# google/automl

Measured on NVIDIA H100. Metric: EfficientDet-D0 images/sec @ batch 32/GPU (640x640, forward + post-process), higher is better.
Workload: dtype f16 storage / f32 accumulate

## Files before the change

automl_b200/csrc/mbconv_fused.cu:

```cuda
#include "tc_common.cuh"

namespace edet {
namespace mbf {

using namespace pwtc;

constexpr int kThreads = 256;
constexpr int kPatch = 16;
constexpr int kPatchPx = kPatch * kPatch;
constexpr int kMaxCh = 64;
constexpr int kNT = kMaxCh / 16;
constexpr int kEPitch = kMaxCh * 2 + 16;

__device__ __forceinline__ uint32_t lds_b32(uint32_t addr) {
  uint32_t v;
  asm volatile("ld.shared.b32 %0, [%1];" : "=r"(v) : "r"(addr));
  return v;
}
__device__ __forceinline__ void sts_v4(uint32_t addr, const uint4& v) {
  asm volatile("st.shared.v4.b32 [%0], {%1, %2, %3, %4};" ::"r"(addr), "r"(v.x), "r"(v.y),
               "r"(v.z), "r"(v.w)
               : "memory");
}
__device__ __forceinline__ float2 h2_bits_to_f2(uint32_t v) {
  return __half22float2(*reinterpret_cast<const __half2*>(&v));
}

struct Params {
  int n, h, w, cin, cmid, ho, wo, pad_t, pad_l;
  int block_k, num_k_blocks, a_bytes, b_bytes, desc_sbo, desc_layout;
  int ch, num_chunks;
  int oth, otw;
  int tiles_y, tiles_x, total_tiles;
  const float* bias_e;
  const float* wd;
  const float* bias_d;
  __half* out;
  long long* se_sum;
  unsigned* sched;
};

struct Tile {
  int n, ty, tx, chunk;
};
__device__ __forceinline__ Tile decode(int t, const Params& p) {
  Tile r;
  r.chunk = t % p.num_chunks;
  t /= p.num_chunks;
  r.tx = t % p.tiles_x;
  t /= p.tiles_x;
  r.ty = t % p.tiles_y;
  r.n = t / p.tiles_y;
  return r;
}

template <int K, int S, int ACT, bool HAS_SE>
__global__ void __launch_bounds__(kThreads, 2)
mbconv_front_kernel(const __grid_constant__ CUtensorMap map_x,
                    const __grid_constant__ CUtensorMap map_w, const Params p) {
  constexpr int OTW = (kPatch - K) / S + 1;
  constexpr int NIX = (OTW - 1) * S + K;
  pdl_launch_dependents();
  extern __shared__ __align__(1024) uint8_t smem_raw[];
  uint8_t* smem = reinterpret_cast<uint8_t*>(
      (reinterpret_cast<uintptr_t>(smem_raw) + 1023) & ~static_cast<uintptr_t>(1023));
  uint8_t* smem_a = smem;
  uint8_t* smem_b = smem_a + p.a_bytes;
  uint8_t* smem_e = smem_b + p.b_bytes;
  unsigned long long* se_s =
      reinterpret_cast<unsigned long long*>(smem_e + kPatchPx * kEPitch);
  uint64_t* bars = reinterpret_cast<uint64_t*>(se_s + p.ch);
  const uint32_t full_bar = smem_u32(bars);
  volatile int* next_tile_s = reinterpret_cast<volatile int*>(bars + 1);

  const int warp = threadIdx.x >> 5, lane = threadIdx.x & 31;
  const int wg = warp >> 2;
  if (threadIdx.x == 0) {
    mbar_init(full_bar, 1);
    asm volatile("fence.mbarrier_init.release.cluster;" ::: "memory");
    asm volatile("prefetch.tensormap [%0];" ::"l"(reinterpret_cast<uint64_t>(&map_x)) : "memory");
    asm volatile("prefetch.tensormap [%0];" ::"l"(reinterpret_cast<uint64_t>(&map_w)) : "memory");
  }
  __syncthreads();
  pdl_wait_prior();

  const uint32_t tx_bytes = static_cast<uint32_t>(kPatchPx * p.block_k * 2 + p.ch * p.block_k * 2);
  const int pitch = p.block_k * 2;
  const int nt = p.ch >> 4;
  uint32_t full_phase = 0;

  auto issue_loads = [&](const Tile& tl, int kb) {
    mbar_expect_tx(full_bar, tx_bytes);
    tma_load_4d(smem_u32(smem_a), &map_x, full_bar, kb * p.block_k, tl.tx * OTW * S - p.pad_l,
                tl.ty * OTW * S - p.pad_t, tl.n);
    tma_load_3d(smem_u32(smem_b), &map_w, full_bar, kb * p.block_k, tl.chunk * p.ch, 0);
  };

  bool prefetched = false;
  int t = blockIdx.x;
  for (int it = 0; t < p.total_tiles; ++it) {
    const Tile tl = decode(t, p);
    const int cbase = tl.chunk * p.ch;
    const int cv = min(p.ch, p.cmid - cbase);
    float acc[2][kNT][8] = {};
    for (int kb = 0; kb < p.num_k_blocks; ++kb) {
      if (threadIdx.x == 0 && !(kb == 0 && prefetched)) issue_loads(tl, kb);
      mbar_wait(full_bar, full_phase);
      full_phase ^= 1;
      const int k_rem = p.cin - kb * p.block_k;
      const int ksteps = k_rem >= p.block_k ? p.block_k / MMA_K : (k_rem + MMA_K - 1) / MMA_K;
      const uint64_t db = make_smem_desc(smem_u32(smem_b), p.desc_sbo, p.desc_layout);
      wg_fence();
#pragma unroll
      for (int h = 0; h < 2; ++h) {
        const uint64_t da =
            make_smem_desc(smem_u32(smem_a + (wg * 128 + h * 64) * pitch), p.desc_sbo, p.desc_layout);
        wg_mma_kblock<kNT>(acc[h], da, db, pitch, nt, ksteps, kb == 0);
      }
      wg_commit();
      wg_wait<0>();
      __syncthreads();
    }
    wg_fence_acc<kNT>(acc[0]);
    wg_fence_acc<kNT>(acc[1]);
    if (threadIdx.x == 0) {
      const int tn = sched_next_tile(p.sched, p.total_tiles);
      next_tile_s[it & 1] = tn;
      prefetched = tn < p.total_tiles;
      if (prefetched) issue_loads(decode(tn, p), 0);
    }
    {
      const int cq = 2 * (lane & 3);
      const float* be = p.bias_e + cbase;
#pragma unroll
      for (int h = 0; h < 2; ++h) {
#pragma unroll
        for (int r = 0; r < 2; ++r) {
          const int m = wg * 128 + h * 64 + 16 * (warp & 3) + (lane >> 2) + 8 * r;
          const int py = m / kPatch, px = m % kPatch;
          const int iy = tl.ty * OTW * S - p.pad_t + py, ix = tl.tx * OTW * S - p.pad_l + px;
          const bool inside = iy >= 0 && iy < p.h && ix >= 0 && ix < p.w;
          const uint32_t erow = smem_u32(smem_e) + m * kEPitch;
#pragma unroll
          for (int j = 0; j < kNT; ++j) {
            const int col = 16 * j + cq;
            if (16 * j >= cv) continue;
            const bool hi_ok = 16 * j + 8 < cv;
            uint32_t lo_bits = 0u, hi_bits = 0u;
            if (inside) {
              const float2 b_lo = __ldg(reinterpret_cast<const float2*>(be + col));
              const float2 b_hi = hi_ok ? __ldg(reinterpret_cast<const float2*>(be + col + 8))
                                        : make_float2(0.f, 0.f);
              float2 lo = fadd2_rn(make_float2(acc[h][j][2 * r], acc[h][j][2 * r + 1]), b_lo);
              float2 hi = fadd2_rn(make_float2(acc[h][j][4 + 2 * r], acc[h][j][4 + 2 * r + 1]), b_hi);
              apply_act4<ACT>(lo, hi);
              const __half2 l2 = __floats2half2_rn(lo.x, lo.y), h2 = __floats2half2_rn(hi.x, hi.y);
              lo_bits = *reinterpret_cast<const uint32_t*>(&l2);
              hi_bits = *reinterpret_cast<const uint32_t*>(&h2);
            }
            asm volatile("st.shared.b32 [%0], %1;" ::"r"(erow + col * 2), "r"(lo_bits) : "memory");
            if (hi_ok)
              asm volatile("st.shared.b32 [%0], %1;" ::"r"(erow + (col + 8) * 2), "r"(hi_bits) : "memory");
          }
        }
      }
      if (HAS_SE)
        for (int i = threadIdx.x; i < p.ch; i += kThreads) se_s[i] = 0ull;
    }
    __syncthreads();
    {
      const int cpn = cv >> 1;
      const int oy0 = tl.ty * OTW, ox0 = tl.tx * OTW;
      const int rows = min(OTW, p.ho - oy0), cols = min(OTW, p.wo - ox0);
      const int cm2 = p.cmid >> 1;
      const uint32_t e_u32 = smem_u32(smem_e);
      if constexpr (K == 3 && S == 2) {
        constexpr int CG = 2;
        constexpr int NCG = (OTW + CG - 1) / CG;
        constexpr int IN_R = (OTW - 1) * S + K, IN_C = (CG - 1) * S + K;
        for (int item = threadIdx.x; item < NCG * cpn; item += kThreads) {
          const int xg = item / cpn, cp = item - xg * cpn;
          const float2* wd2 = reinterpret_cast<const float2*>(p.wd) + ((cbase >> 1) + cp);
          float2 wk[K * K];
#pragma unroll
          for (int i = 0; i < K * K; ++i) wk[i] = __ldg(wd2 + i * cm2);
          uint32_t coff[IN_C];
#pragma unroll
          for (int j = 0; j < IN_C; ++j)
            coff[j] = e_u32 + static_cast<uint32_t>(min(xg * CG * S + j, kPatch - 1) * kEPitch + cp * 4);
          float2 acc[OTW][CG];
#pragma unroll
          for (int r = 0; r < OTW; ++r)
#pragma unroll
            for (int tx = 0; tx < CG; ++tx) acc[r][tx] = make_float2(0.f, 0.f);
#pragma unroll
          for (int ir = 0; ir < IN_R; ++ir) {
            float2 xv[IN_C];
#pragma unroll
            for (int j = 0; j < IN_C; ++j) xv[j] = h2_bits_to_f2(lds_b32(coff[j] + ir * kPatch * kEPitch));
#pragma unroll
            for (int r = 0; r < OTW; ++r) {
              const int ky = ir - r * S;
              if (ky >= 0 && ky < K) {
#pragma unroll
                for (int tx = 0; tx < CG; ++tx)
#pragma unroll
                  for (int kx = 0; kx < K; ++kx)
                    acc[r][tx] = ffma2_rn(xv[tx * S + kx], wk[ky * K + kx], acc[r][tx]);
              }
            }
          }
          const float2 bd = __ldg(reinterpret_cast<const float2*>(p.bias_d + cbase) + cp);
          __half2* ocol = reinterpret_cast<__half2*>(p.out) +
                          ((static_cast<size_t>(tl.n) * p.ho + oy0) * p.wo + ox0 + xg * CG) * cm2 +
                          (cbase >> 1) + cp;
          float2 ssum = make_float2(0.f, 0.f);
#pragma unroll
          for (int r = 0; r < OTW; ++r) {
            float2 o0 = fadd2_rn(acc[r][0], bd), o1 = fadd2_rn(acc[r][1], bd);
            apply_act4<ACT>(o0, o1);
            if (r < rows) {
              if (xg * CG < cols) {
                if (HAS_SE) ssum = fadd2_rn(ssum, o0);
                ocol[static_cast<size_t>(r) * p.wo * cm2] = __floats2half2_rn(o0.x, o0.y);
              }
              if (xg * CG + 1 < cols) {
                if (HAS_SE) ssum = fadd2_rn(ssum, o1);
                ocol[static_cast<size_t>(r) * p.wo * cm2 + cm2] = __floats2half2_rn(o1.x, o1.y);
              }
            }
          }
          if (HAS_SE) {
            atomicAdd(&se_s[2 * cp], static_cast<unsigned long long>(__float2ll_rn(ssum.x * 1048576.f)));
            atomicAdd(&se_s[2 * cp + 1], static_cast<unsigned long long>(__float2ll_rn(ssum.y * 1048576.f)));
          }
        }
      } else {
      for (int item = threadIdx.x; item < rows * cpn; item += kThreads) {
        const int oyl = item / cpn, cp = item - oyl * cpn;
        const float2* wd2 = reinterpret_cast<const float2*>(p.wd) + ((cbase >> 1) + cp);
        const uint32_t ebase = e_u32 + (oyl * S * kPatch) * kEPitch + cp * 4;
        float2 acc[OTW];
#pragma unroll
        for (int i = 0; i < OTW; ++i) acc[i] = make_float2(0.f, 0.f);
#pragma unroll
        for (int ky = 0; ky < K; ++ky) {
          float2 wk[K];
#pragma unroll
          for (int kx = 0; kx < K; ++kx) wk[kx] = __ldg(wd2 + (ky * K + kx) * cm2);
#pragma unroll
          for (int ixl = 0; ixl < NIX; ++ixl) {
            const float2 v = h2_bits_to_f2(lds_b32(ebase + (ky * kPatch + ixl) * kEPitch));
#pragma unroll
            for (int kx = 0; kx < K; ++kx) {
              if ((ixl - kx) >= 0 && (ixl - kx) % S == 0 && (ixl - kx) / S < OTW)
                acc[(ixl - kx) / S] = ffma2_rn(v, wk[kx], acc[(ixl - kx) / S]);
            }
          }
        }
        const float2 bd = __ldg(reinterpret_cast<const float2*>(p.bias_d + cbase) + cp);
        __half2* orow = reinterpret_cast<__half2*>(p.out) +
                        ((static_cast<size_t>(tl.n) * p.ho + oy0 + oyl) * p.wo + ox0) * cm2 +
                        (cbase >> 1) + cp;
#pragma unroll
        for (int i = 0; i < OTW; ++i) acc[i] = fadd2_rn(acc[i], bd);
#pragma unroll
        for (int i = 0; i + 1 < OTW; i += 2) apply_act4<ACT>(acc[i], acc[i + 1]);
        if (OTW & 1) acc[OTW - 1] = apply_act2<ACT>(acc[OTW - 1]);
        float2 ssum = make_float2(0.f, 0.f);
#pragma unroll
        for (int oxl = 0; oxl < OTW; ++oxl) {
          if (oxl < cols) {
            if (HAS_SE) ssum = fadd2_rn(ssum, acc[oxl]);
            orow[static_cast<size_t>(oxl) * cm2] = __floats2half2_rn(acc[oxl].x, acc[oxl].y);
          }
        }
        if (HAS_SE) {
          atomicAdd(&se_s[2 * cp], static_cast<unsigned long long>(__float2ll_rn(ssum.x * 1048576.f)));
          atomicAdd(&se_s[2 * cp + 1], static_cast<unsigned long long>(__float2ll_rn(ssum.y * 1048576.f)));
        }
      }
      }
      if (HAS_SE) {
        __syncthreads();
        unsigned long long* dst = reinterpret_cast<unsigned long long*>(p.se_sum) +
                                  static_cast<size_t>(tl.n) * p.cmid + cbase;
        for (int i = threadIdx.x; i < cv; i += kThreads)
          if (se_s[i] != 0ull) atomicAdd(dst + i, se_s[i]);
      }
    }
    __syncthreads();
    t = next_tile_s[it & 1];
  }
}

template <int K, int S>
static int launch(const CUtensorMap& mx, const CUtensorMap& mw, const Params& p, int grid,
                  int smem_bytes, int act, bool has_se, cudaStream_t stream) {
#define EDET_MBF(ACT, SE)                                                                     \
  do {                                                                                        \
    auto kern = mbconv_front_kernel<K, S, ACT, SE>;                                           \
    static int configured[kMaxDevices];                                                       \
    if (int rc = ensure_dynamic_smem(kern, 232448, configured)) return rc;                    \
    EDET_CHECK_CUDA(launch_pdl(kern, dim3(grid), dim3(kThreads), smem_bytes, stream, mx, mw, p)); \
    return EDET_OK;                                                                           \
  } while (0)
  if (act == EDET_ACT_SWISH && has_se) EDET_MBF(EDET_ACT_SWISH, true);
  if (act == EDET_ACT_SWISH && !has_se) EDET_MBF(EDET_ACT_SWISH, false);
  if (act == EDET_ACT_RELU6 && has_se) EDET_MBF(EDET_ACT_RELU6, true);
  if (act == EDET_ACT_RELU6 && !has_se) EDET_MBF(EDET_ACT_RELU6, false);
#undef EDET_MBF
  set_error("mbconv_expand_dw: unsupported activation %d", act);
  return EDET_ERR_UNSUPPORTED;
}

}
}

extern "C" int edet_mbconv_expand_dw(const edet_half* x, const edet_half* we, const float* bias_e,
                                     const float* wd, const float* bias_d, edet_half* out,
                                     int64_t* se_sum, int n, int h, int w, int cin, int cmid,
                                     int k, int stride, int act, edet_stream_t stream) {
  using namespace edet;
  using namespace edet::mbf;
  EDET_CHECK_ARG(x && we && bias_e && wd && bias_d && out, "mbconv_expand_dw: null pointer");
  EDET_CHECK_ARG(n > 0 && h > 0 && w > 0 && cin % 8 == 0 && cmid % 8 == 0,
                 "mbconv_expand_dw: cin %% 8 and cmid %% 8 required (got %d, %d)", cin, cmid);
  EDET_CHECK_ARG((k == 3 || k == 5) && (stride == 1 || stride == 2), "mbconv_expand_dw: k/stride");
  Params p;
  p.n = n; p.h = h; p.w = w; p.cin = cin; p.cmid = cmid;
  p.ho = ceil_div(h, stride); p.wo = ceil_div(w, stride);
  p.pad_t = same_pad_before(h, k, stride); p.pad_l = same_pad_before(w, k, stride);
  p.num_chunks = ceil_div(cmid, kMaxCh);
  p.ch = ((ceil_div(cmid, p.num_chunks) + 15) / 16) * 16;
  p.oth = p.otw = (kPatch - k) / stride + 1;
  p.tiles_y = ceil_div(p.ho, p.oth); p.tiles_x = ceil_div(p.wo, p.otw);
  p.total_tiles = n * p.tiles_y * p.tiles_x * p.num_chunks;
  int smem_bytes = 0;
  for (int bk = cin <= 16 ? 16 : (cin <= 32 ? 32 : 64); bk >= 16; bk >>= 1) {
    p.block_k = bk;
    p.a_bytes = kPatchPx * bk * 2;
    p.b_bytes = ((p.ch * bk * 2 + 1023) / 1024) * 1024;
    smem_bytes = 1024 + p.a_bytes + p.b_bytes + kPatchPx * kEPitch + p.ch * 8 + 64;
    if (smem_bytes <= 113 * 1024 || bk == 32) break;
  }
  p.num_k_blocks = ceil_div(cin, p.block_k);
  p.desc_layout = desc_layout_for(p.block_k);
  p.desc_sbo = 8 * p.block_k * 2;
  p.bias_e = bias_e; p.bias_d = bias_d;
  p.wd = wd;
  p.out = reinterpret_cast<__half*>(out);
  p.se_sum = reinterpret_cast<long long*>(se_sum);
  p.sched = next_sched_slot();
  if (!p.sched) return EDET_ERR_CUDA;
  EDET_CHECK_ARG(smem_bytes <= 232448, "mbconv_expand_dw: tile needs %d bytes of smem", smem_bytes);
  CUtensorMap mx, mw;
  int rc;
  if ((rc = make_map4(&mx, x, cin, w, h, n, p.block_k, kPatch, kPatch))) return rc;
  if ((rc = make_map(&mw, we, cin, cmid, 1, cin, static_cast<uint64_t>(cmid) * cin, p.ch, p.block_k)))
    return rc;
  const int sm_count = device_sm_count();
  if (!sm_count) return EDET_ERR_CUDA;
  int per_sm = 232448 / (smem_bytes + 1024);
  if (per_sm < 1) per_sm = 1;
  if (per_sm > 2) per_sm = 2;
  const int grid = p.total_tiles < per_sm * sm_count ? p.total_tiles : per_sm * sm_count;
  const bool has_se = se_sum != nullptr;
  cudaStream_t s = as_stream(stream);
  if (k == 3 && stride == 1) return launch<3, 1>(mx, mw, p, grid, smem_bytes, act, has_se, s);
  if (k == 3 && stride == 2) return launch<3, 2>(mx, mw, p, grid, smem_bytes, act, has_se, s);
  if (k == 5 && stride == 1) return launch<5, 1>(mx, mw, p, grid, smem_bytes, act, has_se, s);
  return launch<5, 2>(mx, mw, p, grid, smem_bytes, act, has_se, s);
}
```

automl_b200/engine.py:

```python
import math
import os

import numpy as np
import torch

from automl_b200 import anchors as anchors_lib
from automl_b200 import ops
from automl_b200 import utils
from automl_b200.arch import DetArch


def _round_up(x, m):
  return (x + m - 1) // m * m


def _bn_fold(w, scope, eps):
  g = np.asarray(w[scope + '/gamma'], np.float64)
  b = np.asarray(w[scope + '/beta'], np.float64)
  m = np.asarray(w[scope + '/moving_mean'], np.float64)
  v = np.asarray(w[scope + '/moving_variance'], np.float64)
  scale = g / np.sqrt(v + eps)
  return scale, b - m * scale


def nms_v5_params(nms_configs):
  method = nms_configs['method']
  if method == 'hard' or not method:
    sigma = 0.0
    iou_thresh = nms_configs['iou_thresh'] or 0.5
    score_thresh = nms_configs['score_thresh'] or float('-inf')
  elif method == 'gaussian':
    sigma = nms_configs['sigma'] or 0.5
    iou_thresh = 0.5
    score_thresh = nms_configs['score_thresh'] or 0.001
  else:
    raise ValueError('Inference has invalid nms method {}'.format(method))
  return iou_thresh, score_thresh, sigma / 2


class Engine(object):

  def __init__(self, config, weights, batch_size, device='cuda:0', pw_impl=ops.PW_TCGEN05,
               use_cuda_graph=True, image_id_base=0, fuse_mbconv_front=False,
               fuse_sepconv=True, pipeline=True, defer_heads=False,
               fuse_class_argmax=True):
    if not torch.cuda.is_available():
      raise RuntimeError('automl_b200.Engine needs a CUDA device; there is no CPU fallback')
    self.config = config
    self.arch = a = DetArch(config)
    self.n = int(batch_size)
    self.device = torch.device(device)
    self.pw_impl = pw_impl
    self.use_cuda_graph = use_cuda_graph
    self.image_id_base = image_id_base
    if os.environ.get('EDET_FUSE_FRONT'):
      fuse_mbconv_front = os.environ['EDET_FUSE_FRONT'] != '0'
    self.fuse_mbconv_front = fuse_mbconv_front
    self.fuse_sepconv = fuse_sepconv
    if os.environ.get('EDET_PIPELINE'):
      pipeline = os.environ['EDET_PIPELINE'] != '0'
    self.pipeline = pipeline
    if os.environ.get('EDET_DEFER_HEADS'):
      defer_heads = os.environ['EDET_DEFER_HEADS'] != '0'
    self.defer_heads = bool(defer_heads and pipeline)
    self._deferred = None
    if os.environ.get('EDET_FUSE_ARGMAX'):
      fuse_class_argmax = os.environ['EDET_FUSE_ARGMAX'] != '0'
    self.fuse_class_argmax = fuse_class_argmax
    self._fused_target = None
    self._logits_current = False
    self.act = utils.activation_code(a.act_type)
    self._graph = None
    self._bb_split = None
    self._cell0_end = None
    self._ops = []
    self.op_info = []
    self._branch = None
    self._branch_streams = {}
    self.buffers = {}
    self._keep = []
    self.launches_per_forward = 0
    with torch.cuda.device(self.device):
      self._build(weights)

  def _dev(self, arr, dtype):
    t = torch.as_tensor(np.ascontiguousarray(arr)).to(dtype).to(self.device).contiguous()
    self._keep.append(t)
    return t

  def _buf(self, name, shape, dtype=torch.float16):
    t = torch.empty(shape, dtype=dtype, device=self.device)
    self.buffers[name] = t
    return t

  def _add(self, name, fn, kind='other', nbytes=0, flops=0, kernels=1, branch=None, needs=None):
    self._ops.append((name, fn))
    if branch is None:
      branch = self._branch
    self.op_info.append({'name': name, 'kind': kind, 'bytes': int(nbytes), 'flops': int(flops),
                         'kernels': int(kernels), 'branch': branch, 'needs': list(needs or [])})

  def _pw(self, name, a, wt, bias, out, act, residual=None, batch=1, rows=None, nout=None,
          branch=None):
    if rows is None:
      rows = a.numel() // (a.shape[-1] * batch)
    impl = self.pw_impl
    k = wt.shape[-1]
    n_out = nout if nout is not None else wt.shape[-2]
    m = rows * batch
    wbatch = wt.shape[0] if wt.dim() == 3 else 1
    nbytes = 2 * (m * k + m * n_out * (2 if residual is not None else 1)) + 2 * wbatch * n_out * k
    self._add(name, lambda: ops.pointwise_conv(a, wt, bias, out, act, residual=residual,
                                               rows=rows, batch=batch, nout=nout, impl=impl),
              kind='pointwise_tc' if impl == ops.PW_TCGEN05 else 'pointwise_simt',
              nbytes=nbytes, flops=2 * m * k * n_out, branch=branch)

  def _build(self, w):
    a, n, act = self.arch, self.n, self.act
    eps = a.bn_eps
    f16, f32 = torch.float16, torch.float32
    H, W = a.image_hw
    self.input = self._buf('input', (n, H, W, 3), f32)

    def check_c(c, what):
      if c % 8:
        raise NotImplementedError('%s has %d channels; the kernels need multiples of 8' % (what, c))

    bb = a.backbone_name
    scale, shift = _bn_fold(w, bb + '/stem/tpu_batch_normalization', eps)
    k = np.asarray(w[bb + '/stem/conv2d/kernel'], np.float64) * scale
    stem_w = self._dev(k.reshape(27, -1), f16)
    stem_b = self._dev(shift, f32)
    h, wd = a.level_hw[1]
    x = self._buf('stem', (n, h, wd, a.stem_filters))
    inp = self.input
    self._add('stem', lambda inp=inp, x=x: ops.stem_conv(inp, x, stem_w, stem_b, act),
              kind='stem', nbytes=12 * n * H * W + 2 * n * h * wd * a.stem_filters,
              flops=2 * 27 * n * h * wd * a.stem_filters)
    cur, cur_hw = x, (h, wd)

    feats = {}
    max_mid = max(b.mid_filters for b in a.blocks)
    se_acc = [self._buf('se_acc%d' % i, (n, max_mid), torch.int64) for i in range(2)]
    for t in se_acc:
      t.zero_()
    se_index = 0
    if any(b.se_filters for b in a.blocks):
      self._add('se_clear', lambda t=se_acc[0]: t.zero_(), kind='memset', nbytes=8 * n * max_mid,
                kernels=0)
    for b in a.blocks:
      scope = '%s/%s' % (bb, b.name)
      check_c(b.input_filters, scope); check_c(b.mid_filters, scope); check_c(b.output_filters, scope)
      h, wd = cur_hw
      x_in = cur
      mid = x_in
      fuse_front = (self.fuse_mbconv_front and b.expand_name and b.kernel_size == 3 and
                    b.stride == 2 and b.input_filters <= 64 and h * wd >= 1600)
      exp_wt = exp_b = None
      if b.expand_name:
        s, sh = _bn_fold(w, '%s/%s' % (scope, b.expand_bn), eps)
        kw = np.asarray(w['%s/%s/kernel' % (scope, b.expand_name)], np.float64)[0, 0]
        exp_wt = self._dev((kw * s).T, f16)
        exp_b = self._dev(sh, f32)
        if not fuse_front:
          mid = self._buf(b.name + '/expand', (n, h, wd, b.mid_filters))
          self._pw(b.name + '/expand', x_in, exp_wt, exp_b, mid, act)
      s, sh = _bn_fold(w, '%s/%s' % (scope, b.dw_bn), eps)
      kd = np.asarray(w[scope + '/depthwise_conv2d/depthwise_kernel'], np.float64)[..., 0]
      dw_w = self._dev((kd * s).reshape(b.kernel_size * b.kernel_size, -1), f32)
      dw_b = self._dev(sh, f32)
      ho, wo = utils.same_pad(h, b.kernel_size, b.stride)[0], utils.same_pad(wd, b.kernel_size, b.stride)[0]
      dwo = self._buf(b.name + '/dw', (n, ho, wo, b.mid_filters))
      partial = None
      if b.se_filters:
        partial = se_acc[se_index % 2].view(-1)[:n * b.mid_filters].view(n, b.mid_filters)
        next_zero = se_acc[(se_index + 1) % 2]
        se_index += 1
      if fuse_front:
        self._add(b.name + '/expand_dw',
                  lambda x_in=x_in, exp_wt=exp_wt, exp_b=exp_b, dwo=dwo, dw_w=dw_w, dw_b=dw_b,
                  partial=partial, b=b:
                  ops.mbconv_expand_dw(x_in, exp_wt, exp_b, dw_w, dw_b, dwo, act, b.kernel_size,
                                       b.stride, partial),
                  kind='mbconv_expand_dw',
                  nbytes=2 * n * (h * wd * b.input_filters + ho * wo * b.mid_filters)
                  + 2 * b.mid_filters * (b.input_filters + b.kernel_size**2)
                  + (8 * partial.numel() if partial is not None else 0),
                  flops=2 * n * b.mid_filters * (h * wd * b.input_filters + b.kernel_size**2 * ho * wo))
      else:
        self._add(b.name + '/dw',
                  lambda mid=mid, dwo=dwo, dw_w=dw_w, dw_b=dw_b, partial=partial, b=b:
                  ops.depthwise_conv(mid, dwo, dw_w, dw_b, act, b.kernel_size, b.stride, partial),
                  kind='depthwise_k%ds%d' % (b.kernel_size, b.stride),
                  nbytes=2 * n * b.mid_filters * (h * wd + ho * wo) + 2 * b.kernel_size**2 * b.mid_filters
                  + (8 * partial.numel() if partial is not None else 0),
                  flops=2 * b.kernel_size**2 * n * b.mid_filters * ho * wo)
      s, sh = _bn_fold(w, '%s/%s' % (scope, b.project_bn), eps)
      kp = np.asarray(w['%s/%s/kernel' % (scope, b.project_name)], np.float64)[0, 0]
      proj_wt = self._dev((kp * s).T, f16)
      proj_b = self._dev(sh, f32)
      y = self._buf(b.name + '/out', (n, ho, wo, b.output_filters))
      res = x_in if b.has_skip else None
      if b.reduction and b.reduction >= a.config.min_level and self._bb_split is None:
        self._bb_split = len(self._ops) + (1 if b.se_filters else 0)
      if b.se_filters:
        w1 = self._dev(np.asarray(w[scope + '/se/conv2d/kernel'], np.float64)[0, 0].T, f32)
        b1 = self._dev(w[scope + '/se/conv2d/bias'], f32)
        w2 = self._dev(np.asarray(w[scope + '/se/conv2d_1/kernel'], np.float64)[0, 0], f32)
        b2 = self._dev(w[scope + '/se/conv2d_1/bias'], f32)
        gate = self._buf(b.name + '/se_gate', (n, b.mid_filters), f32)
        hidden = self._buf(b.name + '/se_hidden', (n, b.se_filters), f32)
        wt_scaled = self._buf(b.name + '/proj_w', (n, b.output_filters, b.mid_filters))
        inv_hw = 1.0 / float(ho * wo)
        self._add(b.name + '/se',
                  lambda partial=partial, inv_hw=inv_hw, w1=w1, b1=b1, w2=w2, b2=b2, gate=gate,
                  proj_wt=proj_wt, wt_scaled=wt_scaled, next_zero=next_zero, hidden=hidden:
                  ops.se_fc(partial, inv_hw, w1, b1, w2, b2, gate, act, proj_wt, wt_scaled,
                            next_zero, hidden),
                  kind='se_fc', nbytes=8 * partial.numel() + 2 * proj_wt.numel() + 2 * wt_scaled.numel(),
                  kernels=2)
        self._pw(b.name + '/project', dwo, wt_scaled, proj_b, y, utils.ACT_NONE, residual=res,
                 batch=n, rows=ho * wo)
      else:
        self._pw(b.name + '/project', dwo, proj_wt, proj_b, y, utils.ACT_NONE, residual=res)
      cur, cur_hw = y, (ho, wo)
      if b.reduction:
        feats[b.reduction] = y

    self.num_backbone_ops = len(self._ops)
    if self._bb_split is None:
      self._bb_split = self.num_backbone_ops
    if self.defer_heads:
      for level in sorted(feats):
        if level >= a.config.min_level:
          src = feats[level]
          dst = self._buf('P%d_copy' % level, tuple(src.shape))
          self._add('feat_copy/P%d' % level, lambda src=src, dst=dst: dst.copy_(src),
                    kind='memcpy', nbytes=4 * src.numel(), kernels=0)
          feats[level] = dst
    self._heads_start = len(self._ops)
# ... 559 lines not shown
```

Baseline: 5237.

## Rework fused expand+depthwise kernel as streaming bands with ring buffer, enable auto fusion

Replaces the 16x16 patch tiling of the fused expand-pointwise + depthwise kernel with vertical strips processed as row bands. A double-buffered TMA pipeline feeds WGMMA, and expanded rows live in a shared-memory ring, so halo rows are not recomputed between bands. The host picks strip width and segment count to fit two CTAs per SM and balance the persistent grid. The engine now defaults to an automatic rule that turns the fusion on for large stride-2 k3 blocks, where previously it was off. This adds complexity and risks slowdowns where the fused path beats separate kernels less often than the rule assumes.

```diff
diff --git a/automl_b200/csrc/mbconv_fused.cu b/automl_b200/csrc/mbconv_fused.cu
--- a/automl_b200/csrc/mbconv_fused.cu
+++ b/automl_b200/csrc/mbconv_fused.cu
@@ -6,32 +6,36 @@
 using namespace pwtc;
 
 constexpr int kThreads = 256;
-constexpr int kPatch = 16;
-constexpr int kPatchPx = kPatch * kPatch;
-constexpr int kMaxCh = 64;
-constexpr int kNT = kMaxCh / 16;
-constexpr int kEPitch = kMaxCh * 2 + 16;
-
-__device__ __forceinline__ uint32_t lds_b32(uint32_t addr) {
-  uint32_t v;
-  asm volatile("ld.shared.b32 %0, [%1];" : "=r"(v) : "r"(addr));
-  return v;
-}
-__device__ __forceinline__ void sts_v4(uint32_t addr, const uint4& v) {
-  asm volatile("st.shared.v4.b32 [%0], {%1, %2, %3, %4};" ::"r"(addr), "r"(v.x), "r"(v.y),
-               "r"(v.z), "r"(v.w)
-               : "memory");
-}
-__device__ __forceinline__ float2 h2_bits_to_f2(uint32_t v) {
-  return __half22float2(*reinterpret_cast<const __half2*>(&v));
-}
+constexpr int kCh = 64;
+constexpr int kNT = kCh / 16;
+constexpr int kBK = 16;
+constexpr int kRowBytes = kBK * 2;
+constexpr int kBlockBytes = 64 * kRowBytes;
+constexpr int kEPitch = kCh * 2 + 16;
+constexpr int kTwoPerSm = 113 * 1024;
+constexpr int kMaxSmem = 232448;
+
+template <int K, int S>
+struct Cfg {
+  static constexpr int TR = (S == 2) ? 4 : (K == 3 ? 8 : 4);
+  static constexpr int TC = (S == 2) ? 2 : 4;
+  static constexpr int NR = TR * S;
+  static constexpr int HALO = K - S;
+  static constexpr int L = NR + HALO;
+  static constexpr int IN_COLS = (TC - 1) * S + K;
+  static constexpr int SW_MAX = S == 2 ? 32 : 64;
+  static constexpr int QMAX = (SW_MAX / TC * (kCh / 2) + kThreads - 1) / kThreads;
+};
 
 struct Params {
   int n, h, w, cin, cmid, ho, wo, pad_t, pad_l;
-  int block_k, num_k_blocks, a_bytes, b_bytes, desc_sbo, desc_layout;
-  int ch, num_chunks;
-  int oth, otw;
-  int tiles_y, tiles_x, total_tiles;
+  int nkb;
+  int sw, iw;
+  float inv_iw;
+  int m_blocks;
+  int a_bytes, w_bytes;
+  int nb;
+  int bands, strips, segs, chunks, total_units;
   const float* bias_e;
   const float* wd;
   const float* bias_d;
@@ -40,268 +44,305 @@
   unsigned* sched;
 };
 
-struct Tile {
-  int n, ty, tx, chunk;
+struct Unit {
+  int n, seg, strip, chunk;
 };
-__device__ __forceinline__ Tile decode(int t, const Params& p) {
-  Tile r;
-  r.chunk = t % p.num_chunks;
-  t /= p.num_chunks;
-  r.tx = t % p.tiles_x;
-  t /= p.tiles_x;
-  r.ty = t % p.tiles_y;
-  r.n = t / p.tiles_y;
+__device__ __forceinline__ Unit decode(int u, const Params& p) {
+  Unit r;
+  r.chunk = u % p.chunks;
+  u /= p.chunks;
+  r.strip = u % p.strips;
+  u /= p.strips;
+  r.seg = u % p.segs;
+  r.n = u / p.segs;
   return r;
+}
+
+__device__ __forceinline__ uint32_t lds_b32(uint32_t addr) {
+  uint32_t v;
+  asm volatile("ld.shared.b32 %0, [%1];" : "=r"(v) : "r"(addr));
+  return v;
+}
+__device__ __forceinline__ void sts_b32(uint32_t addr, uint32_t v) {
+  asm volatile("st.shared.b32 [%0], %1;" ::"r"(addr), "r"(v) : "memory");
 }
 
 template <int K, int S, int ACT, bool HAS_SE>
 __global__ void __launch_bounds__(kThreads, 2)
 mbconv_front_kernel(const __grid_constant__ CUtensorMap map_x,
                     const __grid_constant__ CUtensorMap map_w, const Params p) {
-  constexpr int OTW = (kPatch - K) / S + 1;
-  constexpr int NIX = (OTW - 1) * S + K;
+  using C = Cfg<K, S>;
+  constexpr int TR = C::TR, TC = C::TC, NR = C::NR, HALO = C::HALO, L = C::L;
+  constexpr int IN_COLS = C::IN_COLS;
   pdl_launch_dependents();
   extern __shared__ __align__(1024) uint8_t smem_raw[];
   uint8_t* smem = reinterpret_cast<uint8_t*>(
       (reinterpret_cast<uintptr_t>(smem_raw) + 1023) & ~static_cast<uintptr_t>(1023));
   uint8_t* smem_a = smem;
-  uint8_t* smem_b = smem_a + p.a_bytes;
-  uint8_t* smem_e = smem_b + p.b_bytes;
-  unsigned long long* se_s =
-      reinterpret_cast<unsigned long long*>(smem_e + kPatchPx * kEPitch);
-  uint64_t* bars = reinterpret_cast<uint64_t*>(se_s + p.ch);
-  const uint32_t full_bar = smem_u32(bars);
-  volatile int* next_tile_s = reinterpret_cast<volatile int*>(bars + 1);
-
-  const int warp = threadIdx.x >> 5, lane = threadIdx.x & 31;
+  uint8_t* smem_w = smem_a + 2 * p.a_bytes;
+  uint8_t* smem_e = smem_w + 2 * p.w_bytes;
+  const int ring_row_bytes = p.iw * kEPitch;
+  ulonglong2* se_s = reinterpret_cast<ulonglong2*>(smem_e + L * ring_row_bytes);
+  uint64_t* bars = reinterpret_cast<uint64_t*>(se_s + C::QMAX * kThreads);
+  volatile int* unit_s = reinterpret_cast<volatile int*>(bars + 2);
+
+  const int warp = __shfl_sync(0xffffffffu, static_cast<int>(threadIdx.x >> 5), 0);
+  const int lane = threadIdx.x & 31;
   const int wg = warp >> 2;
   if (threadIdx.x == 0) {
-    mbar_init(full_bar, 1);
+    mbar_init(smem_u32(&bars[0]), 1);
+    mbar_init(smem_u32(&bars[1]), 1);
     asm volatile("fence.mbarrier_init.release.cluster;" ::: "memory");
     asm volatile("prefetch.tensormap [%0];" ::"l"(reinterpret_cast<uint64_t>(&map_x)) : "memory");
     asm volatile("prefetch.tensormap [%0];" ::"l"(reinterpret_cast<uint64_t>(&map_w)) : "memory");
   }
+  pdl_wait_prior();
+
+  auto issue = [&](const Unit& un, int j, int stage, int wbuf) {
+    const uint32_t bar = smem_u32(&bars[stage]);
+    const uint32_t a_tx = static_cast<uint32_t>(p.nkb * NR * p.iw * kRowBytes);
+    mbar_expect_tx(bar, a_tx + (wbuf >= 0 ? static_cast<uint32_t>(p.nkb * kBlockBytes) : 0u));
+    const int y0 = (un.seg * p.nb * TR) * S - p.pad_t + HALO + (j - 1) * NR;
+    const int x0 = un.strip * p.sw * S - p.pad_l;
+    uint8_t* dst = smem_a + stage * p.a_bytes;
+    for (int kb = 0; kb < p.nkb; ++kb)
+      tma_load_4d(smem_u32(dst + kb * p.m_blocks * kBlockBytes), &map_x, bar, kb * kBK, x0, y0, un.n);
+    if (wbuf >= 0)
+      for (int kb = 0; kb < p.nkb; ++kb)
+        tma_load_3d(smem_u32(smem_w + wbuf * p.w_bytes + kb * kBlockBytes), &map_w, bar, kb * kBK,
+                    un.chunk * kCh, 0);
+  };
+  auto bands_of = [&](const Unit& un) { return min(p.nb, p.bands - un.seg * p.nb); };
+
+  if (threadIdx.x == 0) {
+    const int u0 = static_cast<int>(blockIdx.x);
+    unit_s[0] = u0;
+    issue(decode(u0, p), 0, 0, 0);
+  }
   __syncthreads();
-  pdl_wait_prior();
-
-  const uint32_t tx_bytes = static_cast<uint32_t>(kPatchPx * p.block_k * 2 + p.ch * p.block_k * 2);
-  const int pitch = p.block_k * 2;
-  const int nt = p.ch >> 4;
-  uint32_t full_phase = 0;
-
-  auto issue_loads = [&](const Tile& tl, int kb) {
-    mbar_expect_tx(full_bar, tx_bytes);
-    tma_load_4d(smem_u32(smem_a), &map_x, full_bar, kb * p.block_k, tl.tx * OTW * S - p.pad_l,
-                tl.ty * OTW * S - p.pad_t, tl.n);
-    tma_load_3d(smem_u32(smem_b), &map_w, full_bar, kb * p.block_k, tl.chunk * p.ch, 0);
-  };
-
-  bool prefetched = false;
-  int t = blockIdx.x;
-  for (int it = 0; t < p.total_tiles; ++it) {
-    const Tile tl = decode(t, p);
-    const int cbase = tl.chunk * p.ch;
-    const int cv = min(p.ch, p.cmid - cbase);
-    float acc[2][kNT][8] = {};
-    for (int kb = 0; kb < p.num_k_blocks; ++kb) {
-      if (threadIdx.x == 0 && !(kb == 0 && prefetched)) issue_loads(tl, kb);
-      mbar_wait(full_bar, full_phase);
-      full_phase ^= 1;
-      const int k_rem = p.cin - kb * p.block_k;
-      const int ksteps = k_rem >= p.block_k ? p.block_k / MMA_K : (k_rem + MMA_K - 1) / MMA_K;
-      const uint64_t db = make_smem_desc(smem_u32(smem_b), p.desc_sbo, p.desc_layout);
-      wg_fence();
-#pragma unroll
-      for (int h = 0; h < 2; ++h) {
-        const uint64_t da =
-            make_smem_desc(smem_u32(smem_a + (wg * 128 + h * 64) * pitch), p.desc_sbo, p.desc_layout);
-        wg_mma_kblock<kNT>(acc[h], da, db, pitch, nt, ksteps, kb == 0);
+
+  const uint32_t e_u32 = smem_u32(smem_e);
+  const int cm2 = p.cmid >> 1;
+  const int nmt = p.sw / TC;
+  int g = 0;
+  for (int ui = 0;; ++ui) {
+    const int u = __shfl_sync(0xffffffffu, unit_s[ui & 1], 0);
+    if (u >= p.total_units) break;
+    const Unit un = decode(u, p);
+    const int nchunks = bands_of(un) + 1;
+    const int cbase = un.chunk * kCh;
+    const int cv = min(kCh, p.cmid - cbase);
+    const int cpn = cv >> 1;
+    const int n_items = nmt * cpn;
+    const int seg_oy0 = un.seg * p.nb * TR;
+    const int ws = seg_oy0 * S - p.pad_t;
+    const int sx0 = un.strip * p.sw * S - p.pad_l;
+    const uint8_t* w_tile = smem_w + (ui & 1) * p.w_bytes;
+    if (HAS_SE)
+      for (int q = 0; q < C::QMAX; ++q) se_s[q * kThreads + threadIdx.x] = make_ulonglong2(0ull, 0ull);
+    float2 bias_lo[kNT], bias_hi[kNT];
+#pragma unroll
+    for (int jn = 0; jn < kNT; ++jn) {
+      const int col = 16 * jn + 2 * (lane & 3);
+      bias_lo[jn] = col < cv ? __ldg(reinterpret_cast<const float2*>(p.bias_e + cbase + col)) : make_float2(0.f, 0.f);
+      bias_hi[jn] = col + 8 < cv ? __ldg(reinterpret_cast<const float2*>(p.bias_e + cbase + col + 8))
+                                 : make_float2(0.f, 0.f);
+    }
+
+    for (int j = 0; j < nchunks; ++j, ++g) {
+      if (threadIdx.x == 0) {
+        if (j + 1 < nchunks) {
+          issue(un, j + 1, (g + 1) & 1, -1);
+        } else {
+          const int un_next = sched_next_tile(p.sched, p.total_units);
+          unit_s[(ui + 1) & 1] = un_next;
+          if (un_next < p.total_units) issue(decode(un_next, p), 0, (g + 1) & 1, (ui + 1) & 1);
+        }
       }
-      wg_commit();
-      wg_wait<0>();
-      __syncthreads();
-    }
-    wg_fence_acc<kNT>(acc[0]);
-    wg_fence_acc<kNT>(acc[1]);
-    if (threadIdx.x == 0) {
-      const int tn = sched_next_tile(p.sched, p.total_tiles);
-      next_tile_s[it & 1] = tn;
-      prefetched = tn < p.total_tiles;
-      if (prefetched) issue_loads(decode(tn, p), 0);
-    }
-    {
-      const int cq = 2 * (lane & 3);
-      const float* be = p.bias_e + cbase;
-#pragma unroll
-      for (int h = 0; h < 2; ++h) {
+      mbar_wait(smem_u32(&bars[g & 1]), static_cast<uint32_t>(g >> 1) & 1u);
+      const uint8_t* a_tile = smem_a + (g & 1) * p.a_bytes;
+      const int m_valid = NR * p.iw;
+      const int row_lo = j == 0 ? NR - HALO : 0;
+      for (int mb = wg; mb < p.m_blocks; mb += 2) {
+        float acc[kNT][8] = {};
+        wg_fence();
+        for (int kb = 0; kb < p.nkb; ++kb) {
+          const uint64_t da = make_smem_desc(smem_u32(a_tile + (kb * p.m_blocks + mb) * kBlockBytes), 8 * kRowBytes, 3);
+          const uint64_t db = make_smem_desc(smem_u32(w_tile + kb * kBlockBytes), 8 * kRowBytes, 3);
+          wg_mma_kblock_wide<kNT>(acc, da, db, 1, kb == 0);
+        }
+        wg_commit();
+        wg_wait<0>();
+        wg_fence_acc<kNT>(acc);
+        const int cq = 2 * (lane & 3);
 #pragma unroll
         for (int r = 0; r < 2; ++r) {
-          const int m = wg * 128 + h * 64 + 16 * (warp & 3) + (lane >> 2) + 8 * r;
-          const int py = m / kPatch, px = m % kPatch;
-          const int iy = tl.ty * OTW * S - p.pad_t + py, ix = tl.tx * OTW * S - p.pad_l + px;
+          const int m = mb * 64 + 16 * (warp & 3) + (lane >> 2) + 8 * r;
+          if (m >= m_valid) continue;
+          const int lr = __float2int_rz(__fmul_rn(static_cast<float>(m) + 0.5f, p.inv_iw));
+          const int x = m - lr * p.iw;
+          if (lr < row_lo) continue;
+          const int iy_rel = HALO + (j - 1) * NR + lr;
+          const int iy = ws + iy_rel, ix = sx0 + x;
           const bool inside = iy >= 0 && iy < p.h && ix >= 0 && ix < p.w;
-          const uint32_t erow = smem_u32(smem_e) + m * kEPitch;
-#pragma unroll
-          for (int j = 0; j < kNT; ++j) {
-            const int col = 16 * j + cq;
-            if (16 * j >= cv) continue;
-            const bool hi_ok = 16 * j + 8 < cv;
+          const uint32_t epix = e_u32 + static_cast<uint32_t>((iy_rel % L) * ring_row_bytes + x * kEPitch);
+#pragma unroll
+          for (int jn = 0; jn < kNT; ++jn) {
+            const int col = 16 * jn + cq;
+            if (16 * jn >= cv) continue;
+            const bool hi_ok = 16 * jn + 8 < cv;
             uint32_t lo_bits = 0u, hi_bits = 0u;
             if (inside) {
-              const float2 b_lo = __ldg(reinterpret_cast<const float2*>(be + col));
-              const float2 b_hi = hi_ok ? __ldg(reinterpret_cast<const float2*>(be + col + 8))
-                                        : make_float2(0.f, 0.f);
-              float2 lo = fadd2_rn(make_float2(acc[h][j][2 * r], acc[h][j][2 * r + 1]), b_lo);
-              float2 hi = fadd2_rn(make_float2(acc[h][j][4 + 2 * r], acc[h][j][4 + 2 * r + 1]), b_hi);
+              float2 lo = fadd2_rn(make_float2(acc[jn][2 * r], acc[jn][2 * r + 1]), bias_lo[jn]);
+              float2 hi = fadd2_rn(make_float2(acc[jn][4 + 2 * r], acc[jn][4 + 2 * r + 1]), bias_hi[jn]);
               apply_act4<ACT>(lo, hi);
               const __half2 l2 = __floats2half2_rn(lo.x, lo.y), h2 = __floats2half2_rn(hi.x, hi.y);
               lo_bits = *reinterpret_cast<const uint32_t*>(&l2);
               hi_bits = *reinterpret_cast<const uint32_t*>(&h2);
             }
-            asm volatile("st.shared.b32 [%0], %1;" ::"r"(erow + col * 2), "r"(lo_bits) : "memory");
-            if (hi_ok)
-              asm volatile("st.shared.b32 [%0], %1;" ::"r"(erow + (col + 8) * 2), "r"(hi_bits) : "memory");
+            sts_b32(epix + col * 2, lo_bits);
+            if (hi_ok) sts_b32(epix + (col + 8) * 2, hi_bits);
           }
         }
       }
-      if (HAS_SE)
-        for (int i = threadIdx.x; i < p.ch; i += kThreads) se_s[i] = 0ull;
-    }
-    __syncthreads();
-    {
-      const int cpn = cv >> 1;
-      const int oy0 = tl.ty * OTW, ox0 = tl.tx * OTW;
-      const int rows = min(OTW, p.ho - oy0), cols = min(OTW, p.wo - ox0);
-      const int cm2 = p.cmid >> 1;
-      const uint32_t e_u32 = smem_u32(smem_e);
-      if constexpr (K == 3 && S == 2) {
-        constexpr int CG = 2;
-        constexpr int NCG = (OTW + CG - 1) / CG;
-        constexpr int IN_R = (OTW - 1) * S + K, IN_C = (CG - 1) * S + K;
-        for (int item = threadIdx.x; item < NCG * cpn; item += kThreads) {
-          const int xg = item / cpn, cp = item - xg * cpn;
-          const float2* wd2 = reinterpret_cast<const float2*>(p.wd) + ((cbase >> 1) + cp);
-          float2 wk[K * K];
-#pragma unroll
-          for (int i = 0; i < K * K; ++i) wk[i] = __ldg(wd2 + i * cm2);
-          uint32_t coff[IN_C];
-#pragma unroll
-          for (int j = 0; j < IN_C; ++j)
-            coff[j] = e_u32 + static_cast<uint32_t>(min(xg * CG * S + j, kPatch - 1) * kEPitch + cp * 4);
-          float2 acc[OTW][CG];
-#pragma unroll
-          for (int r = 0; r < OTW; ++r)
-#pragma unroll
-            for (int tx = 0; tx < CG; ++tx) acc[r][tx] = make_float2(0.f, 0.f);
-#pragma unroll
-          for (int ir = 0; ir < IN_R; ++ir) {
-            float2 xv[IN_C];
-#pragma unroll
-            for (int j = 0; j < IN_C; ++j) xv[j] = h2_bits_to_f2(lds_b32(coff[j] + ir * kPatch * kEPitch));
-#pragma unroll
-            for (int r = 0; r < OTW; ++r) {
-              const int ky = ir - r * S;
-              if (ky >= 0 && ky < K) {
-#pragma unroll
-                for (int tx = 0; tx < CG; ++tx)
-#pragma unroll
-                  for (int kx = 0; kx < K; ++kx)
-                    acc[r][tx] = ffma2_rn(xv[tx * S + kx], wk[ky * K + kx], acc[r][tx]);
+      __syncthreads();
+      if (j == 0) continue;
+      const int b = j - 1;
+      const int oy0 = seg_oy0 + b * TR;
+      const int slot0 = (b * NR) % L;
+#pragma unroll 1
+      for (int q = 0; q < C::QMAX; ++q) {
+        const int item = static_cast<int>(threadIdx.x) + q * kThreads;
+        if (item >= n_items) break;
+        const int mt = item / cpn, cp = item - mt * cpn;
+        const int ox0 = un.strip * p.sw + mt * TC;
+        const float2* wd2 = reinterpret_cast<const float2*>(p.wd) + ((cbase >> 1) + cp);
+        float2 wreg[K * K];
+#pragma unroll
+        for (int t = 0; t < K * K; ++t) wreg[t] = __ldg(wd2 + t * cm2);
+        const uint32_t cbyte = e_u32 + static_cast<uint32_t>(mt * TC * S * kEPitch + cp * 4);
+        float2 acc[TR][TC];
+#pragma unroll
+        for (int r = 0; r < TR; ++r)
+#pragma unroll
+          for (int tx = 0; tx < TC; ++tx) acc[r][tx] = make_float2(0.f, 0.f);
+#pragma unroll
+        for (int ir = 0; ir < L; ++ir) {
+          const int slot = slot0 + ir < L ? slot0 + ir : slot0 + ir - L;
+          const uint32_t rbase = cbyte + static_cast<uint32_t>(slot * ring_row_bytes);
+          float2 xv[IN_COLS];
+#pragma unroll
+          for (int c = 0; c < IN_COLS; ++c) {
+            const uint32_t raw = lds_b32(rbase + c * kEPitch);
+            xv[c] = __half22float2(*reinterpret_cast<const __half2*>(&raw));
+          }
+#pragma unroll
+          for (int r = 0; r < TR; ++r) {
+            const int ky = ir - r * S;
+            if (ky >= 0 && ky < K) {
+#pragma unroll
+              for (int tx = 0; tx < TC; ++tx)
+#pragma unroll
+                for (int kx = 0; kx < K; ++kx)
+                  acc[r][tx] = ffma2_rn(xv[tx * S + kx], wreg[ky * K + kx], acc[r][tx]);
+            }
+          }
+        }
+        const float2 bv = __ldg(reinterpret_cast<const float2*>(p.bias_d + cbase) + cp);
+        __half2* orow = reinterpret_cast<__half2*>(p.out) +
+                        ((static_cast<size_t>(un.n) * p.ho + oy0) * p.wo + ox0) * cm2 + (cbase >> 1) + cp;
+        float2 ssum = make_float2(0.f, 0.f);
+#pragma unroll
+        for (int r = 0; r < TR; ++r) {
+          if (oy0 + r < p.ho) {
+            float2 o[TC];
+#pragma unroll
+            for (int tx = 0; tx < TC; ++tx) o[tx] = fadd2_rn(acc[r][tx], bv);
+#pragma unroll
+            for (int tx = 0; tx + 1 < TC; tx += 2) apply_act4<ACT>(o[tx], o[tx + 1]);
+#pragma unroll
+            for (int tx = 0; tx < TC; ++tx) {
+              if (ox0 + tx < p.wo) {
+                if (HAS_SE) ssum = fadd2_rn(ssum, o[tx]);
+                orow[static_cast<size_t>(tx) * cm2] = __floats2half2_rn(o[tx].x, o[tx].y);
               }
             }
           }
-          const float2 bd = __ldg(reinterpret_cast<const float2*>(p.bias_d + cbase) + cp);
-          __half2* ocol = reinterpret_cast<__half2*>(p.out) +
-                          ((static_cast<size_t>(tl.n) * p.ho + oy0) * p.wo + ox0 + xg * CG) * cm2 +
-                          (cbase >> 1) + cp;
-          float2 ssum = make_float2(0.f, 0.f);
-#pragma unroll
-          for (int r = 0; r < OTW; ++r) {
-            float2 o0 = fadd2_rn(acc[r][0], bd), o1 = fadd2_rn(acc[r][1], bd);
-            apply_act4<ACT>(o0, o1);
-            if (r < rows) {
-              if (xg * CG < cols) {
-                if (HAS_SE) ssum = fadd2_rn(ssum, o0);
-                ocol[static_cast<size_t>(r) * p.wo * cm2] = __floats2half2_rn(o0.x, o0.y);
-              }
-              if (xg * CG + 1 < cols) {
-                if (HAS_SE) ssum = fadd2_rn(ssum, o1);
-                ocol[static_cast<size_t>(r) * p.wo * cm2 + cm2] = __floats2half2_rn(o1.x, o1.y);
-              }
-            }
-          }
-          if (HAS_SE) {
-            atomicAdd(&se_s[2 * cp], static_cast<unsigned long long>(__float2ll_rn(ssum.x * 1048576.f)));
-            atomicAdd(&se_s[2 * cp + 1], static_cast<unsigned long long>(__float2ll_rn(ssum.y * 1048576.f)));
-          }
-        }
-      } else {
-      for (int item = threadIdx.x; item < rows * cpn; item += kThreads) {
-        const int oyl = item / cpn, cp = item - oyl * cpn;
-        const float2* wd2 = reinterpret_cast<const float2*>(p.wd) + ((cbase >> 1) + cp);
-        const uint32_t ebase = e_u32 + (oyl * S * kPatch) * kEPitch + cp * 4;
-        float2 acc[OTW];
-#pragma unroll
-        for (int i = 0; i < OTW; ++i) acc[i] = make_float2(0.f, 0.f);
-#pragma unroll
-        for (int ky = 0; ky < K; ++ky) {
-          float2 wk[K];
-#pragma unroll
-          for (int kx = 0; kx < K; ++kx) wk[kx] = __ldg(wd2 + (ky * K + kx) * cm2);
-#pragma unroll
-          for (int ixl = 0; ixl < NIX; ++ixl) {
-            const float2 v = h2_bits_to_f2(lds_b32(ebase + (ky * kPatch + ixl) * kEPitch));
-#pragma unroll
-            for (int kx = 0; kx < K; ++kx) {
-              if ((ixl - kx) >= 0 && (ixl - kx) % S == 0 && (ixl - kx) / S < OTW)
-                acc[(ixl - kx) / S] = ffma2_rn(v, wk[kx], acc[(ixl - kx) / S]);
-            }
-          }
-        }
-        const float2 bd = __ldg(reinterpret_cast<const float2*>(p.bias_d + cbase) + cp);
-        __half2* orow = reinterpret_cast<__half2*>(p.out) +
-                        ((static_cast<size_t>(tl.n) * p.ho + oy0 + oyl) * p.wo + ox0) * cm2 +
-                        (cbase >> 1) + cp;
-#pragma unroll
-        for (int i = 0; i < OTW; ++i) acc[i] = fadd2_rn(acc[i], bd);
-#pragma unroll
-        for (int i = 0; i + 1 < OTW; i += 2) apply_act4<ACT>(acc[i], acc[i + 1]);
-        if (OTW & 1) acc[OTW - 1] = apply_act2<ACT>(acc[OTW - 1]);
-        float2 ssum = make_float2(0.f, 0.f);
-#pragma unroll
-        for (int oxl = 0; oxl < OTW; ++oxl) {
-          if (oxl < cols) {
-            if (HAS_SE) ssum = fadd2_rn(ssum, acc[oxl]);
-            orow[static_cast<size_t>(oxl) * cm2] = __floats2half2_rn(acc[oxl].x, acc[oxl].y);
-          }
+          orow += static_cast<size_t>(p.wo) * cm2;
         }
         if (HAS_SE) {
-          atomicAdd(&se_s[2 * cp], static_cast<unsigned long long>(__float2ll_rn(ssum.x * 1048576.f)));
-          atomicAdd(&se_s[2 * cp + 1], static_cast<unsigned long long>(__float2ll_rn(ssum.y * 1048576.f)));
+          ulonglong2& v = se_s[q * kThreads + threadIdx.x];
+          v.x += static_cast<unsigned long long>(__float2ll_rn(ssum.x * 1048576.f));
+          v.y += static_cast<unsigned long long>(__float2ll_rn(ssum.y * 1048576.f));
         }
       }
-      }
-      if (HAS_SE) {
-        __syncthreads();
-        unsigned long long* dst = reinterpret_cast<unsigned long long*>(p.se_sum) +
-                                  static_cast<size_t>(tl.n) * p.cmid + cbase;
-        for (int i = threadIdx.x; i < cv; i += kThreads)
-          if (se_s[i] != 0ull) atomicAdd(dst + i, se_s[i]);
+      __syncthreads();
+    }
+    if (HAS_SE) {
+      unsigned long long* dst = reinterpret_cast<unsigned long long*>(p.se_sum) +
+                                static_cast<size_t>(un.n) * p.cmid + cbase;
+      for (int q = 0; q < C::QMAX; ++q) {
+        const int item = static_cast<int>(threadIdx.x) + q * kThreads;
+        if (item < n_items) {
+          const int cp = item % cpn;
+          const ulonglong2 v = se_s[q * kThreads + threadIdx.x];
+          if (v.x != 0ull) atomicAdd(dst + 2 * cp, v.x);
+          if (v.y != 0ull) atomicAdd(dst + 2 * cp + 1, v.y);
+        }
       }
     }
-    __syncthreads();
-    t = next_tile_s[it & 1];
   }
 }
 
 template <int K, int S>
-static int launch(const CUtensorMap& mx, const CUtensorMap& mw, const Params& p, int grid,
-                  int smem_bytes, int act, bool has_se, cudaStream_t stream) {
+static int run(const __half* x, const __half* we, Params& p, int act, bool has_se,
+               cudaStream_t stream) {
+  using C = Cfg<K, S>;
+  p.ho = ceil_div(p.h, S); p.wo = ceil_div(p.w, S);
+  p.pad_t = same_pad_before(p.h, K, S); p.pad_l = same_pad_before(p.w, K, S);
+  p.nkb = ceil_div(p.cin, kBK);
+  p.chunks = ceil_div(p.cmid, kCh);
+  p.w_bytes = p.nkb * kBlockBytes;
+  int smem_bytes = 0;
+  for (p.sw = C::SW_MAX;; p.sw >>= 1) {
+    p.iw = (p.sw - 1) * S + K;
+    p.inv_iw = 1.0f / static_cast<float>(p.iw);
+    p.m_blocks = ceil_div(C::NR * p.iw, 64);
+    p.a_bytes = p.nkb * p.m_blocks * kBlockBytes;
+    smem_bytes = 1024 + 2 * p.a_bytes + 2 * p.w_bytes + C::L * p.iw * kEPitch +
+                 C::QMAX * kThreads * 16 + 2 * 8 + 2 * 4;
+    if (smem_bytes <= kTwoPerSm || p.sw <= 2 * C::TC) break;
+  }
+  EDET_CHECK_ARG(smem_bytes <= kMaxSmem, "mbconv_expand_dw: cin %d needs %d bytes of smem", p.cin,
+                 smem_bytes);
+  const int per_sm = smem_bytes <= kTwoPerSm ? 2 : 1;
+  const int sms = device_sm_count();
+  if (!sms) return EDET_ERR_CUDA;
+  int grid = per_sm * std::max(1, sms - option_persist_slack());
+  p.strips = ceil_div(p.wo, p.sw);
+  p.bands = ceil_div(p.ho, C::TR);
+  const long long base = static_cast<long long>(p.n) * p.strips * p.chunks;
+  const int nb_min = ceil_div(20 * C::HALO, C::NR);
+  long long segs = (4LL * grid + base - 1) / base;
+  segs = std::min<long long>(segs, std::max(1, p.bands / nb_min));
+  p.nb = ceil_div(p.bands, static_cast<int>(std::max(1LL, segs)));
+  p.segs = ceil_div(p.bands, p.nb);
+  const long long total = base * p.segs;
+  EDET_CHECK_ARG(total < 0x7fffffffLL, "mbconv_expand_dw: too many work units");
+  p.total_units = static_cast<int>(total);
+  if (grid > p.total_units) grid = p.total_units;
+  p.sched = next_sched_slot();
+  if (!p.sched) return EDET_ERR_CUDA;
+  CUtensorMap mx, mw;
+  int rc;
+  if ((rc = make_map4(&mx, x, p.cin, p.w, p.h, p.n, kBK, p.iw, C::NR))) return rc;
+  if ((rc = make_map(&mw, we, p.cin, p.cmid, 1, p.cin, static_cast<uint64_t>(p.cmid) * p.cin, kCh, kBK)))
+    return rc;
 #define EDET_MBF(ACT, SE)                                                                     \
   do {                                                                                        \
     auto kern = mbconv_front_kernel<K, S, ACT, SE>;                                           \
     static int configured[kMaxDevices];                                                       \
-    if (int rc = ensure_dynamic_smem(kern, 232448, configured)) return rc;                    \
+    if (int rc2 = ensure_dynamic_smem(kern, kMaxSmem, configured)) return rc2;                \
     EDET_CHECK_CUDA(launch_pdl(kern, dim3(grid), dim3(kThreads), smem_bytes, stream, mx, mw, p)); \
     return EDET_OK;                                                                           \
   } while (0)
@@ -329,46 +370,15 @@
   EDET_CHECK_ARG((k == 3 || k == 5) && (stride == 1 || stride == 2), "mbconv_expand_dw: k/stride");
   Params p;
   p.n = n; p.h = h; p.w = w; p.cin = cin; p.cmid = cmid;
-  p.ho = ceil_div(h, stride); p.wo = ceil_div(w, stride);
-  p.pad_t = same_pad_before(h, k, stride); p.pad_l = same_pad_before(w, k, stride);
-  p.num_chunks = ceil_div(cmid, kMaxCh);
-  p.ch = ((ceil_div(cmid, p.num_chunks) + 15) / 16) * 16;
-  p.oth = p.otw = (kPatch - k) / stride + 1;
-  p.tiles_y = ceil_div(p.ho, p.oth); p.tiles_x = ceil_div(p.wo, p.otw);
-  p.total_tiles = n * p.tiles_y * p.tiles_x * p.num_chunks;
-  int smem_bytes = 0;
-  for (int bk = cin <= 16 ? 16 : (cin <= 32 ? 32 : 64); bk >= 16; bk >>= 1) {
-    p.block_k = bk;
-    p.a_bytes = kPatchPx * bk * 2;
-    p.b_bytes = ((p.ch * bk * 2 + 1023) / 1024) * 1024;
-    smem_bytes = 1024 + p.a_bytes + p.b_bytes + kPatchPx * kEPitch + p.ch * 8 + 64;
-    if (smem_bytes <= 113 * 1024 || bk == 32) break;
-  }
-  p.num_k_blocks = ceil_div(cin, p.block_k);
-  p.desc_layout = desc_layout_for(p.block_k);
-  p.desc_sbo = 8 * p.block_k * 2;
-  p.bias_e = bias_e; p.bias_d = bias_d;
-  p.wd = wd;
+  p.bias_e = bias_e; p.bias_d = bias_d; p.wd = wd;
   p.out = reinterpret_cast<__half*>(out);
   p.se_sum = reinterpret_cast<long long*>(se_sum);
-  p.sched = next_sched_slot();
-  if (!p.sched) return EDET_ERR_CUDA;
-  EDET_CHECK_ARG(smem_bytes <= 232448, "mbconv_expand_dw: tile needs %d bytes of smem", smem_bytes);
-  CUtensorMap mx, mw;
-  int rc;
-  if ((rc = make_map4(&mx, x, cin, w, h, n, p.block_k, kPatch, kPatch))) return rc;
-  if ((rc = make_map(&mw, we, cin, cmid, 1, cin, static_cast<uint64_t>(cmid) * cin, p.ch, p.block_k)))
-    return rc;
-  const int sm_count = device_sm_count();
-  if (!sm_count) return EDET_ERR_CUDA;
-  int per_sm = 232448 / (smem_bytes + 1024);
-  if (per_sm < 1) per_sm = 1;
-  if (per_sm > 2) per_sm = 2;
-  const int grid = p.total_tiles < per_sm * sm_count ? p.total_tiles : per_sm * sm_count;
   const bool has_se = se_sum != nullptr;
+  const __half* xh = reinterpret_cast<const __half*>(x);
+  const __half* wh = reinterpret_cast<const __half*>(we);
   cudaStream_t s = as_stream(stream);
-  if (k == 3 && stride == 1) return launch<3, 1>(mx, mw, p, grid, smem_bytes, act, has_se, s);
-  if (k == 3 && stride == 2) return launch<3, 2>(mx, mw, p, grid, smem_bytes, act, has_se, s);
-  if (k == 5 && stride == 1) return launch<5, 1>(mx, mw, p, grid, smem_bytes, act, has_se, s);
-  return launch<5, 2>(mx, mw, p, grid, smem_bytes, act, has_se, s);
-}
+  if (k == 3 && stride == 1) return run<3, 1>(xh, wh, p, act, has_se, s);
+  if (k == 3 && stride == 2) return run<3, 2>(xh, wh, p, act, has_se, s);
+  if (k == 5 && stride == 1) return run<5, 1>(xh, wh, p, act, has_se, s);
+  return run<5, 2>(xh, wh, p, act, has_se, s);
+}
diff --git a/automl_b200/engine.py b/automl_b200/engine.py
--- a/automl_b200/engine.py
+++ b/automl_b200/engine.py
@@ -21,6 +21,24 @@
   v = np.asarray(w[scope + '/moving_variance'], np.float64)
   scale = g / np.sqrt(v + eps)
   return scale, b - m * scale
+
+
+def dw_tiled(h, w, c, k, stride):
+  toh, tow = {(3, 1): (16, 16), (3, 2): (8, 8), (5, 1): (8, 16), (5, 2): (8, 8)}[(k, stride)]
+  ho, wo = -(-h // stride), -(-w // stride)
+  covered = -(-ho // toh) * toh * (-(-wo // tow) * tow)
+  return c >= 64 and ho * wo * 10 >= covered * 7
+
+
+FUSE_FRONT_MIN_BYTES = 256 << 20
+
+
+def fuse_mbconv_front_rule(block, batch, h, w):
+  if not block.expand_name or block.kernel_size != 3 or block.stride != 2:
+    return False
+  if 2 * batch * h * w * block.mid_filters <= FUSE_FRONT_MIN_BYTES:
+    return False
+  return dw_tiled(h, w, block.mid_filters, block.kernel_size, block.stride)
 
 
 def nms_v5_params(nms_configs):
@@ -41,7 +59,7 @@
 class Engine(object):
 
   def __init__(self, config, weights, batch_size, device='cuda:0', pw_impl=ops.PW_TCGEN05,
-               use_cuda_graph=True, image_id_base=0, fuse_mbconv_front=False,
+               use_cuda_graph=True, image_id_base=0, fuse_mbconv_front=None,
                fuse_sepconv=True, pipeline=True, defer_heads=False,
                fuse_class_argmax=True):
     if not torch.cuda.is_available():
@@ -53,8 +71,9 @@
     self.pw_impl = pw_impl
     self.use_cuda_graph = use_cuda_graph
     self.image_id_base = image_id_base
-    if os.environ.get('EDET_FUSE_FRONT'):
-      fuse_mbconv_front = os.environ['EDET_FUSE_FRONT'] != '0'
+    env = os.environ.get('EDET_FUSE_FRONT')
+    if env:
+      fuse_mbconv_front = None if env == 'auto' else env != '0'
     self.fuse_mbconv_front = fuse_mbconv_front
     self.fuse_sepconv = fuse_sepconv
     if os.environ.get('EDET_PIPELINE'):
@@ -154,8 +173,11 @@
       h, wd = cur_hw
       x_in = cur
       mid = x_in
-      fuse_front = (self.fuse_mbconv_front and b.expand_name and b.kernel_size == 3 and
-                    b.stride == 2 and b.input_filters <= 64 and h * wd >= 1600)
+      if self.fuse_mbconv_front is None:
+        fuse_front = fuse_mbconv_front_rule(b, n, h, wd)
+      else:
+        fuse_front = bool(self.fuse_mbconv_front and b.expand_name and
+                          dw_tiled(h, wd, b.mid_filters, b.kernel_size, b.stride))
       exp_wt = exp_b = None
       if b.expand_name:
         s, sh = _bn_fold(w, '%s/%s' % (scope, b.expand_bn), eps)
```

Measured after the change: 5417, median of 6. 1.03x the previous value.
